# rayanirban/DiffSplitting

Hardware: AMD Instinct MI355X
Metric: sampled images/sec (2000-step 128x128 SR3) (higher is better)
Workload: dtype bf16; 1 GPU; sr_sr3_16_128: GaussianDiffusion.p_sample_loop, 16->128 SR3 UNet (97.8M params), T=2000 linear schedule; one step = UNet forward + posterior update of the batch; batch_per_gpu=16, global_batch=16, image=128x128x3, sample_steps=2000, parallelism=1 independent replicas, final RCCL all-gather, hipgraph=True, streams=1, noise=device Philox4x32-10, weights=random-init, seed 0

## Files before the change

diffsplitting_amd/csrc/dsx_attn.hip:

```cpp
#include "dsx_kernels.h"
#include <type_traits>
#include <utility>

namespace dsx {

typedef __attribute__((ext_vector_type(16))) float f32x16;
typedef __attribute__((ext_vector_type(8))) __bf16 bf16x8_a;
typedef __attribute__((ext_vector_type(8))) _Float16 f16x8_a;

namespace {

template <class F, int... I>
__device__ __forceinline__ __attribute__((always_inline)) void attn_static_for_impl(F&& f, std::integer_sequence<int, I...>) {
  (f(std::integral_constant<int, I>{}), ...);
}
template <int N, class F> __device__ __forceinline__ void attn_static_for(F&& f) {
  attn_static_for_impl(f, std::make_integer_sequence<int, N>{});
}

constexpr int BQ = 32;
constexpr int BK = 128;

template <int ST> struct AttnT;
template <> struct AttnT<0> {
  static constexpr int ES = 4;
  static constexpr int DC = 64;
  static constexpr int VK = 64;
};
template <> struct AttnT<1> { static constexpr int ES = 2; static constexpr int DC = 128; static constexpr int VK = 128; };
template <> struct AttnT<2> { static constexpr int ES = 2; static constexpr int DC = 128; static constexpr int VK = 128; };

__device__ __forceinline__ unsigned pack16(float lo, float hi, std::integral_constant<int, 1>) {
  const __bf16 l = (__bf16)lo, h = (__bf16)hi;
  return (unsigned)__builtin_bit_cast(unsigned short, l) | ((unsigned)__builtin_bit_cast(unsigned short, h) << 16);
}
__device__ __forceinline__ unsigned pack16(float lo, float hi, std::integral_constant<int, 2>) {
  const _Float16 l = (_Float16)lo, h = (_Float16)hi;
  return (unsigned)__builtin_bit_cast(unsigned short, l) | ((unsigned)__builtin_bit_cast(unsigned short, h) << 16);
}

template <int ST>
__device__ __forceinline__ f32x16 mfma16(const uint4 a, const uint4 b, f32x16 c) {
  if constexpr (ST == 1)
    return __builtin_amdgcn_mfma_f32_32x32x16_bf16(__builtin_bit_cast(bf16x8_a, a), __builtin_bit_cast(bf16x8_a, b), c, 0, 0, 0);
  else
    return __builtin_amdgcn_mfma_f32_32x32x16_f16(__builtin_bit_cast(f16x8_a, a), __builtin_bit_cast(f16x8_a, b), c, 0, 0, 0);
}

__device__ __forceinline__ int vt_slot(int row, int slot) { return slot ^ (((row >> 3) ^ row) & 15); }

}

template <int ST, int NDB, int CS>
__global__ __launch_bounds__(256, (NDB <= 1 ? 2 : 1)) void k_attn(const AttnArgs a) {
  static_assert(NDB % CS == 0, "whole chunks per workgroup");
  constexpr int NDO = NDB / CS;
  using T = AttnT<ST>;
  constexpr int ES = T::ES, DC = T::DC, VK = T::VK;
  constexpr bool F32 = ST == 0;
  constexpr int KUNITS = NDB * (128 / DC);
  constexpr int VPC = BK / VK;
  constexpr int VUNITS = NDO * VPC;
  constexpr int KROW = F32 ? (DC + 1) * 4 : DC * 2 + 16;
  constexpr int PROW = F32 ? (BK + 1) * 4 : BK * 2 + 16;
  constexpr int VROW = F32 ? 128 * 4 : BK * 2;
  constexpr int KV_BYTES = (BK * KROW > (F32 ? VK : 128) * VROW) ? BK * KROW : (F32 ? VK : 128) * VROW;
  constexpr int Q_BYTES = BQ * KROW;
  constexpr int P_BYTES = BQ * PROW;

  extern __shared__ __attribute__((aligned(16))) unsigned char smem[];
  unsigned char* kv_lds = smem;
  unsigned char* q_lds = smem + KV_BYTES;
  unsigned char* p_lds = q_lds + Q_BYTES;
  float* red = (float*)(p_lds + P_BYTES);

  const int tid = threadIdx.x, lane = tid & 63;
  const int wave = __builtin_amdgcn_readfirstlane(tid >> 6);
  const int li = lane & 31, lh = lane >> 5;

  const int QT = (a.L + BQ - 1) / BQ;
  const int total = a.B * QT * CS;
  int j = blockIdx.x;
  if ((total & 7) == 0) j = (blockIdx.x & 7) * (total >> 3) + (blockIdx.x >> 3);
  const int half = CS == 1 ? 0 : j % CS;
  const int jq = CS == 1 ? j : j / CS;
  const int b = jq / QT, q0 = (jq - b * QT) * BQ;
  const int chunk0 = half * NDO;

  const size_t row0 = (size_t)b * a.L;
  const size_t ldb = (size_t)a.ld * ES;

  constexpr int SEGS = (DC * ES) / 16;
  static_assert(SEGS == 16, "a staged K/Q row is 256 bytes");
  const int seg = tid & 15, rsub = tid >> 4;
#ifndef DSX_ATTN_PD
#define DSX_ATTN_PD 2
#endif
  constexpr int PD = (KUNITS + VUNITS) < DSX_ATTN_PD ? (KUNITS + VUNITS) : DSX_ATTN_PD;
  uint4 pre[PD][10];

  const __amdgpu_buffer_rsrc_t rs = __builtin_amdgcn_make_buffer_rsrc(
      (void*)((const char*)a.q + row0 * ldb), 0, (int)((size_t)a.L * ldb), 0x00020000);
  const unsigned koff = (unsigned)((const char*)a.k - (const char*)a.q), voff = (unsigned)((const char*)a.v - (const char*)a.q);
  auto ld16 = [&](unsigned tensor_off, int row, int col_elem) __attribute__((always_inline)) -> uint4 {
    const unsigned vo = col_elem < a.C ? (unsigned)row * (unsigned)ldb + tensor_off + (unsigned)col_elem * ES : 0x80000000u;
    return __builtin_bit_cast(uint4, __builtin_amdgcn_raw_buffer_load_b128(rs, vo, 0, 0));
  };

  auto issue_unit = [&](int key0, int u, uint4 (&pre)[10]) __attribute__((always_inline)) {
    if (u < KUNITS) {
      const int c0 = u * DC + seg * (16 / ES);
#pragma unroll
      for (int it = 0; it < 8; ++it) {
        const int key = key0 + rsub + 16 * it;
        pre[it] = ld16(koff, key, c0);
      }
#pragma unroll
      for (int it = 0; it < 2; ++it) {
        const int q = q0 + rsub + 16 * it;
        pre[8 + it] = ld16(0u, q, c0);
      }
    } else {
      const int v = u - KUNITS, chunk = v / VPC, part = v - chunk * VPC;
      if constexpr (F32) {
        const int s32 = tid & 31, r8 = tid >> 5;
        const int c0 = (chunk0 + chunk) * 128 + s32 * 4;
#pragma unroll
        for (int it = 0; it < 8; ++it) {
          const int key = key0 + part * VK + r8 + 8 * it;
          pre[it] = ld16(voff, key, c0);
        }
      } else {
        const int c0 = (chunk0 + chunk) * 128 + seg * 8;
#pragma unroll
        for (int it = 0; it < 4; ++it) {
          const int key = key0 + 2 * (rsub + 16 * it);
          pre[2 * it] = ld16(voff, key, c0);
          pre[2 * it + 1] = ld16(voff, key + 1, c0);
        }
      }
    }
  };
  auto store_unit = [&](int u, const uint4 (&pre)[10]) __attribute__((always_inline)) {
    if (u < KUNITS) {
      auto put = [&](unsigned char* dst, const uint4 v) __attribute__((always_inline)) {
        if constexpr (F32) {
          unsigned* d = (unsigned*)dst;
          d[0] = v.x; d[1] = v.y; d[2] = v.z; d[3] = v.w;
        } else {
          *(uint4*)dst = v;
        }
      };
#pragma unroll
      for (int it = 0; it < 8; ++it) put(kv_lds + (rsub + 16 * it) * KROW + seg * 16, pre[it]);
#pragma unroll
      for (int it = 0; it < 2; ++it) put(q_lds + (rsub + 16 * it) * KROW + seg * 16, pre[8 + it]);
    } else {
      if constexpr (F32) {
        const int s32 = tid & 31, r8 = tid >> 5;
#pragma unroll
        for (int it = 0; it < 8; ++it) *(uint4*)(kv_lds + (r8 + 8 * it) * VROW + s32 * 16) = pre[it];
      } else {
#pragma unroll
        for (int it = 0; it < 4; ++it) {
          const int pair = rsub + 16 * it;
          const unsigned ea[4] = {pre[2 * it].x, pre[2 * it].y, pre[2 * it].z, pre[2 * it].w};
          const unsigned eb[4] = {pre[2 * it + 1].x, pre[2 * it + 1].y, pre[2 * it + 1].z, pre[2 * it + 1].w};
#pragma unroll
          for (int jj = 0; jj < 8; ++jj) {
            const unsigned lo = (jj & 1) ? (ea[jj >> 1] >> 16) : (ea[jj >> 1] & 0xffffu);
            const unsigned hi = (jj & 1) ? (eb[jj >> 1] & 0xffff0000u) : (eb[jj >> 1] << 16);
            const int row = seg * 8 + jj;
            *(unsigned*)(kv_lds + row * VROW + vt_slot(row, pair >> 2) * 16 + (pair & 3) * 4) = lo | hi;
          }
        }
      }
    }
  };

  f32x16 oacc[NDO];
#pragma unroll
  for (int c = 0; c < NDO; ++c)
#pragma unroll
    for (int r = 0; r < 16; ++r) oacc[c][r] = 0.f;
  float m_run = -INFINITY, l_run = 0.f;
  f32x16 sacc;

  const int ntiles = (a.L + BK - 1) / BK;
  constexpr int UPT = KUNITS + VUNITS;
  static_assert(UPT % PD == 0 && UPT >= PD, "the register slot of a unit is a compile-time constant");
  attn_static_for<PD>([&](auto pc) __attribute__((always_inline)) {
    constexpr int u0 = decltype(pc)::value;
    issue_unit(0, u0, pre[u0]);
  });
  for (int t = 0; t < ntiles; ++t) {
    const int key0 = t * BK;
#pragma unroll
    for (int r = 0; r < 16; ++r) sacc[r] = 0.f;
    attn_static_for<UPT>([&](auto uc) __attribute__((always_inline)) {
      constexpr int u = decltype(uc)::value;
      __syncthreads();
      store_unit(u, pre[u % PD]);
      __syncthreads();
      {
        constexpr int nu = (u + PD) % UPT;
        const int nk = (u + PD >= UPT) ? key0 + BK : key0;
        if (nk < a.L) issue_unit(nk, nu, pre[u % PD]);
      }
      if constexpr (u < KUNITS) {
        if constexpr (F32) {
          const float* kr = (const float*)(kv_lds + (wave * 32 + li) * KROW);
          const float* qr = (const float*)(q_lds + li * KROW);
#pragma unroll 8
          for (int s = 0; s < DC / 2; ++s)
            sacc = __builtin_amdgcn_mfma_f32_32x32x2f32(kr[2 * s + lh], qr[2 * s + lh], sacc, 0, 0, 0);
        } else {
          const unsigned char* kr = kv_lds + (wave * 32 + li) * KROW + lh * 16;
          const unsigned char* qr = q_lds + li * KROW + lh * 16;
#pragma unroll
          for (int s = 0; s < DC / 16; ++s)
            sacc = mfma16<ST>(*(const uint4*)(kr + s * 32), *(const uint4*)(qr + s * 32), sacc);
        }
        if constexpr (u == KUNITS - 1) {
          float s[16];
          float mx = -INFINITY;
#pragma unroll
          for (int r = 0; r < 16; ++r) {
            const int key = key0 + wave * 32 + (r & 3) + 8 * (r >> 2) + 4 * lh;
            float v = F32 ? sacc[r] / a.div : sacc[r] * a.inv_div;
            if (key >= a.L) v = -INFINITY;
            s[r] = v;
            mx = fmaxf(mx, v);
          }
          mx = fmaxf(mx, __shfl_xor(mx, 32, 64));
          if (lh == 0) red[wave * 32 + li] = mx;
          __syncthreads();
          const float tmax = fmaxf(fmaxf(red[li], red[32 + li]), fmaxf(red[64 + li], red[96 + li]));
          const float m_new = fmaxf(m_run, tmax);
          const float alpha = F32 ? expf(m_run - m_new) : __expf(m_run - m_new);
          float psum = 0.f;
#pragma unroll
          for (int r = 0; r < 16; ++r) { s[r] = F32 ? expf(s[r] - m_new) : __expf(s[r] - m_new); psum += s[r]; }
          psum += __shfl_xor(psum, 32, 64);
          if (lh == 0) red[128 + wave * 32 + li] = psum;
          if constexpr (F32) {
            float* pr = (float*)(p_lds + li * PROW);
#pragma unroll
            for (int r = 0; r < 16; ++r) pr[wave * 32 + (r & 3) + 8 * (r >> 2) + 4 * lh] = s[r];
          } else {
#pragma unroll
            for (int g = 0; g < 4; ++g) {
              uint2 w;
              w.x = pack16(s[4 * g], s[4 * g + 1], std::integral_constant<int, ST>{});
              w.y = pack16(s[4 * g + 2], s[4 * g + 3], std::integral_constant<int, ST>{});
              *(uint2*)(p_lds + li * PROW + (wave * 32 + 8 * g + 4 * lh) * 2) = w;
            }
          }
          __syncthreads();
          const float tsum = (red[128 + li] + red[160 + li]) + (red[192 + li] + red[224 + li]);
          l_run = l_run * alpha + tsum;
          m_run = m_new;
#pragma unroll
          for (int c = 0; c < NDO; ++c)
#pragma unroll
            for (int r = 0; r < 16; ++r) oacc[c][r] *= alpha;
        }
      } else {
        constexpr int v = u - KUNITS, chunk = v / VPC, part = v - chunk * VPC;
        f32x16 acc = oacc[chunk];
        if constexpr (F32) {
          const float* vr = (const float*)kv_lds + wave * 32 + li;
          const float* pr = (const float*)(p_lds + li * PROW) + part * VK;
#pragma unroll 8
          for (int s = 0; s < VK / 2; ++s)
            acc = __builtin_amdgcn_mfma_f32_32x32x2f32(vr[(2 * s + lh) * 128], pr[2 * s + lh], acc, 0, 0, 0);
        } else {
          const int row = wave * 32 + li;
          const unsigned char* vr = kv_lds + row * VROW;
          const unsigned char* pr = p_lds + li * PROW + lh * 16;
#pragma unroll
          for (int s = 0; s < BK / 16; ++s)
            acc = mfma16<ST>(*(const uint4*)(vr + vt_slot(row, 2 * s + lh) * 16), *(const uint4*)(pr + s * 32), acc);
        }
        oacc[chunk] = acc;
      }
    });
  }

  const int q = q0 + li;
  if (q >= a.L) return;
  const float inv_l = 1.0f / l_run;
  char* orow = (char*)a.out + ((size_t)b * a.L + q) * (size_t)a.ldo * ES;
#pragma unroll
  for (int c = 0; c < NDO; ++c) {
#pragma unroll
    for (int g = 0; g < 4; ++g) {
      const int ch = (chunk0 + c) * 128 + wave * 32 + 8 * g + 4 * lh;
      if (ch >= a.C) continue;
      const float x0 = oacc[c][4 * g] * inv_l, x1 = oacc[c][4 * g + 1] * inv_l;
      const float x2 = oacc[c][4 * g + 2] * inv_l, x3 = oacc[c][4 * g + 3] * inv_l;
      if constexpr (F32) {
        *(float4*)(orow + (size_t)ch * 4) = make_float4(x0, x1, x2, x3);
      } else {
        uint2 w;
        w.x = pack16(x0, x1, std::integral_constant<int, ST>{});
        w.y = pack16(x2, x3, std::integral_constant<int, ST>{});
        *(uint2*)(orow + (size_t)ch * 2) = w;
      }
    }
  }
}

namespace {
template <int ST> constexpr size_t attn_lds_bytes() {
  using T = AttnT<ST>;
  constexpr bool F32 = ST == 0;
  constexpr int KROW = F32 ? (T::DC + 1) * 4 : T::DC * 2 + 16;
  constexpr int PROW = F32 ? (BK + 1) * 4 : BK * 2 + 16;
  constexpr int VROW = F32 ? 128 * 4 : BK * 2;
  constexpr int KV = (BK * KROW > (F32 ? T::VK : 128) * VROW) ? BK * KROW : (F32 ? T::VK : 128) * VROW;
  return (size_t)KV + (size_t)BQ * KROW + (size_t)BQ * PROW + 2 * 4 * 32 * sizeof(float);
}
template <int ST, int NDB, int CS = 1> hipError_t launch_attn_one(const AttnArgs& a, hipStream_t st) {
  const int QT = (a.L + BQ - 1) / BQ;
  hipLaunchKernelGGL((k_attn<ST, NDB, CS>), dim3((unsigned)(a.B * QT * CS)), dim3(256), attn_lds_bytes<ST>(), st, a);
  return hipGetLastError();
}
template <int ST> hipError_t launch_attn_st(const AttnArgs& a, bool col_split, hipStream_t st) {
  const int ndb = (a.C + 127) / 128;
  switch (ndb) {
    case 1: return launch_attn_one<ST, 1>(a, st);
    case 2: return launch_attn_one<ST, 2>(a, st);
    case 3: case 4: {
      const int QT = (a.L + BQ - 1) / BQ;
      if (col_split && a.B * QT <= 160) return launch_attn_one<ST, 4, 2>(a, st);
      return launch_attn_one<ST, 4>(a, st);
    }
    case 5: case 6: case 7: case 8: return launch_attn_one<ST, 8>(a, st);
    default: return hipErrorInvalidValue;
  }
}
}

bool attn_supported(int C, int L) { return C >= 8 && C <= 1024 && (C & 7) == 0 && L >= 1 && (long long)L * 3 * C * 4 < (1LL << 31); }

hipError_t launch_attn(const AttnArgs& a, bool col_split, hipStream_t st) {
  if (!attn_supported(a.C, a.L) || a.B < 1) return hipErrorInvalidValue;
  const int epu = a.storage == 0 ? 4 : 8;
  if ((a.ld % epu) || (a.ldo % 4) || ((uintptr_t)a.q & 15) || ((uintptr_t)a.k & 15) || ((uintptr_t)a.v & 15) ||
      ((uintptr_t)a.out & 15))
    return hipErrorInvalidValue;
  switch (a.storage) {
    case 0: return launch_attn_st<0>(a, col_split, st);
    case 1: return launch_attn_st<1>(a, col_split, st);
    case 2: return launch_attn_st<2>(a, col_split, st);
    default: return hipErrorInvalidValue;
  }
}

}
```

diffsplitting_amd/csrc/dsx_exec.cpp:

```cpp
#include "dsx_rt.h"

std::unique_ptr<dsx_exec> dsx::new_exec(dsx_model* m, int B, int H, int W, int cond_channels) {
  auto ex = std::make_unique<dsx_exec>();
  ex->m = m; ex->B = B; ex->H = H; ex->W = W;
  ex->knobs = read_plan_knobs();
  ex->knobs.conv_naive = m->want_naive;
  ex->cond_c = cond_channels; ex->x_c = m->cfg.in_channel - cond_channels;
  return ex;
}

extern "C" int dsx_exec_create(dsx_model* m, int B, int H, int W, int cond_channels, dsx_exec** out) {
  if (!m || !out || B < 1 || H < 1 || W < 1) return fail(DSX_ERR_INVALID, "bad argument");
  if (!m->finalized) return fail(DSX_ERR_STATE, "dsx_model_finalize must precede dsx_exec_create");
  if (cond_channels < 0 || cond_channels >= m->cfg.in_channel) return fail(DSX_ERR_INVALID, "bad cond_channels");
  HIP_TRY(conv_init());
  HIP_TRY(ops_init());
  auto ex = new_exec(m, B, H, W, cond_channels);
  const int rc = run_planner(ex.get(), nullptr, nullptr);
  if (rc) return rc;
  if (hipMemset(ex->step_ctr, 0, 256) != hipSuccess) return fail(DSX_ERR_HIP, "hipMemset failed");
  *out = ex.release();
  return DSX_OK;
}

static int drop_graph(dsx_exec* ex) {
  if (ex->graph.exec && ex->last_stream) HIP_TRY(hipStreamSynchronize(ex->last_stream));
  ex->graph.reset();
  return DSX_OK;
}

extern "C" void dsx_exec_destroy(dsx_exec* ex) {
  if (!ex) return;
  for (auto& sl : ex->staging)
    if (sl.busy) (void)hipEventSynchronize(sl.ev.e);
  (void)drop_graph(ex);
  delete ex;
}
extern "C" size_t dsx_exec_workspace_bytes(const dsx_exec* ex) { return ex ? ex->ws_bytes : 0; }
extern "C" int dsx_exec_handoff_timeouts(dsx_exec* ex, unsigned* count) {
  if (!ex || !count) return fail(DSX_ERR_INVALID, "null argument");
  HIP_TRY(hipDeviceSynchronize());
  HIP_TRY(hipMemcpy(count, ex->handoff_timeouts, sizeof(unsigned), hipMemcpyDeviceToHost));
  return DSX_OK;
}
extern "C" int dsx_exec_num_launches(const dsx_exec* ex) { return ex ? ex->launches : 0; }

extern "C" int dsx_exec_num_ops(const dsx_exec* ex) { return ex ? (int)ex->ops.size() : 0; }
extern "C" int dsx_exec_num_layers(const dsx_exec* ex) { return ex ? (int)ex->layers.size() : 0; }
extern "C" int dsx_exec_layer_info(const dsx_exec* ex, int i, dsx_layer_info* info) {
  if (!ex || !info || i < 0 || i >= (int)ex->layers.size()) return fail(DSX_ERR_INVALID, "bad layer index");
  *info = ex->layers[i];
  return DSX_OK;
}
extern "C" int dsx_exec_copy_workspace(const dsx_exec* ex, uint64_t src, size_t bytes, void* dst, void* stream) {
  if (!ex || !dst) return fail(DSX_ERR_INVALID, "null argument");
  const uint64_t lo = (uint64_t)(uintptr_t)ex->ws, hi = lo + ex->ws_bytes;
  if (!ex->ws || src < lo || src > hi || bytes > hi - src) return fail(DSX_ERR_INVALID, "range is not inside the workspace");
  HIP_TRY(hipMemcpyAsync(dst, (const void*)(uintptr_t)src, bytes, hipMemcpyDeviceToDevice, (hipStream_t)stream));
  return DSX_OK;
}
extern "C" int dsx_exec_op_info(const dsx_exec* ex, int i, char* desc, int cap, int* kind, double* flops,
                                double* bytes) {
  if (!ex || i < 0 || i >= (int)ex->ops.size()) return fail(DSX_ERR_INVALID, "bad op index");
  const PlanOp& o = ex->ops[i];
  if (desc && cap > 0) snprintf(desc, cap, "%s", o.desc.c_str());
  if (kind) *kind = o.kind;
  if (flops) *flops = o.flops;
  if (bytes) *bytes = o.bytes;
  return DSX_OK;
}
extern "C" int dsx_exec_time_kind(dsx_exec* ex, int kind, int iters, float* ms_per_replay, int* launches,
                                  void* stream) {
  if (!ex || !ms_per_replay || iters < 1) return fail(DSX_ERR_INVALID, "bad argument");
  hipStream_t st = (hipStream_t)stream;
  if (!st) return fail(DSX_ERR_INVALID, "dsx_exec_time_kind needs a non-default stream (stream capture)");
  auto selected = [&](int k) { return kind >= 0 ? k == kind : (kind == -1 ? true : k != -kind - 2); };
  int n = 0;
  for (auto& op : ex->ops) n += selected(op.kind) ? 1 : 0;
  if (launches) *launches = n;
  if (n == 0) { *ms_per_replay = 0.f; return DSX_OK; }
  Graph g;
  HIP_TRY(hipStreamSynchronize(st));
  HIP_TRY(hipStreamBeginCapture(st, hipStreamCaptureModeThreadLocal));
  hipError_t err = hipSuccess;
  for (size_t i = 0; i < ex->ops.size() && err == hipSuccess; ++i)
    if (selected(ex->ops[i].kind)) err = launch_op(ex->ops[i], st);
  hipError_t e2 = hipStreamEndCapture(st, &g.graph);
  if (err != hipSuccess || e2 != hipSuccess || !g.graph)
    return fail(DSX_ERR_HIP, "capture of the kernel family failed: %s", hipGetErrorString(err != hipSuccess ? err : e2));
  HIP_TRY(hipGraphInstantiate(&g.exec, g.graph, nullptr, nullptr, 0));
  Event e0, e1;
  HIP_TRY(e0.create());
  HIP_TRY(e1.create());
  HIP_TRY(hipGraphLaunch(g.exec, st));
  HIP_TRY(hipEventRecord(e0.e, st));
  for (int it = 0; it < iters; ++it) HIP_TRY(hipGraphLaunch(g.exec, st));
  HIP_TRY(hipEventRecord(e1.e, st));
  HIP_TRY(hipStreamSynchronize(st));
  float ms = 0.f;
  HIP_TRY(hipEventElapsedTime(&ms, e0.e, e1.e));
  *ms_per_replay = ms / iters;
  return DSX_OK;
}

extern "C" int dsx_exec_read_stamps(dsx_exec* ex, unsigned long long* out128) {
  if (!ex || !out128) return fail(DSX_ERR_INVALID, "null argument");
  memset(out128, 0, 128 * 8);
  if (!ex->stamp_buf) return DSX_OK;
  HIP_TRY(hipDeviceSynchronize());
  HIP_TRY(hipMemcpy(out128, ex->stamp_buf, 128 * 8, hipMemcpyDeviceToHost));
  return DSX_OK;
}

extern "C" int dsx_exec_profile(dsx_exec* ex, int iters, float* ms_per_op, void* stream) {
  if (!ex || !ms_per_op || iters < 1) return fail(DSX_ERR_INVALID, "bad argument");
  hipStream_t st = (hipStream_t)stream;
  const size_t n = ex->ops.size();
  std::vector<Event> ev(2 * n);
  for (auto& e : ev) HIP_TRY(e.create());
  std::vector<double> acc(n, 0.0);
  for (int it = 0; it < iters; ++it) {
    static const bool trace = getenv("DSX_TRACE") != nullptr;
    for (size_t i = 0; i < n; ++i) {
      if (trace) { fprintf(stderr, "[dsx] op %zu: %s\n", i, ex->ops[i].desc.c_str()); fflush(stderr); }
      HIP_TRY(hipEventRecord(ev[2 * i].e, st));
      HIP_TRY(launch_op(ex->ops[i], st));
      HIP_TRY(hipEventRecord(ev[2 * i + 1].e, st));
      if (trace) HIP_TRY(hipStreamSynchronize(st));
    }
    HIP_TRY(hipStreamSynchronize(st));
    for (size_t i = 0; i < n; ++i) {
      float ms = 0.f;
      HIP_TRY(hipEventElapsedTime(&ms, ev[2 * i].e, ev[2 * i + 1].e));
      acc[i] += ms;
    }
  }
  for (size_t i = 0; i < n; ++i) ms_per_op[i] = (float)(acc[i] / iters);
  return DSX_OK;
}

static int run_unet(dsx_exec* ex, bool from_table, int n_time, hipStream_t st, int per_sample = 0) {
  dsx_model* m = ex->m;
  if (m->cfg.with_time_emb) {
    TembArgs t{};
    t.flavour = m->cfg.flavour; t.B = ex->B; t.n_time = n_time;
    t.time = from_table ? nullptr : ex->time_buf;
    t.table = ex->table.as<float>(); t.step_ctr = ex->step_ctr; t.per_sample = per_sample;
    t.inner = m->cfg.inner_channel; t.freq = m->d_freq;
    t.w1 = m->d_w1; t.b1 = m->d_b1; t.w2 = m->d_w2; t.b2 = m->d_b2;
    t.wf = m->d_wf; t.bf = m->d_bf; t.F = m->F; t.film = ex->film;
    HIP_TRY(launch_temb(t, st));
  }
  for (auto& op : ex->ops) HIP_TRY(launch_op(op, st));
  return DSX_OK;
}

static int load_inputs(dsx_exec* ex, const float* cond_nchw, const float* x_nchw, int x_total_c,
                       int x_c_off, hipStream_t st);

extern "C" int dsx_unet_forward(dsx_exec* ex, const float* x, const float* time, int n_time, float* y,
                                void* stream) {
  if (!ex || !x || !y) return fail(DSX_ERR_INVALID, "null argument");
  hipStream_t st = (hipStream_t)stream;
  dsx_model* m = ex->m;
  if (m->cfg.with_time_emb) {
    if (!time || !(n_time == 1 || n_time == ex->B)) return fail(DSX_ERR_INVALID, "n_time must be 1 or B");
    HIP_TRY(hipMemcpyAsync(ex->time_buf, time, (size_t)n_time * 4, hipMemcpyDeviceToDevice, st));
  }
  int rc = load_inputs(ex, ex->cond_c ? x : nullptr, x, m->cfg.in_channel, ex->cond_c, st);
// ... 258 lines not shown
```

diffsplitting_amd/csrc/dsx_kernels.h:

```cpp
#pragma once
#include <hip/hip_runtime.h>
#include <stdint.h>

namespace dsx {

struct PrefetchArgs {
  const void* base;
  unsigned slice_bytes;
  int nslices;
  unsigned* sink;
};
inline unsigned fastdiv_magic(unsigned d) { return d <= 1 ? 0u : (unsigned)((1ull << 32) / d) + 1u; }
#if defined(__HIPCC__)
__device__ __forceinline__ unsigned fastdiv(unsigned n, unsigned magic) { return magic ? __umulhi(n, magic) : n; }
struct PfAcc { unsigned v[4]; };
__device__ __forceinline__ PfAcc l2_prefetch(const PrefetchArgs& pf, unsigned lin_block, unsigned nblocks_total, int tid, int nthreads) {
  PfAcc acc = {{0u, 0u, 0u, 0u}};
  if (pf.base == nullptr || pf.nslices <= 0) return acc;
  const unsigned label = lin_block & 7u, j = lin_block >> 3, n8 = (nblocks_total + 7u) >> 3;
  const unsigned lines = pf.slice_bytes >> 7;
  const unsigned per = (lines + n8 - 1u) / n8, l0 = j * per;
  const unsigned l1 = l0 + per < lines ? l0 + per : lines;
  const int s0 = pf.nslices < 8 ? (int)(label % (unsigned)pf.nslices) : (int)label;
  const int sstep = pf.nslices < 8 ? pf.nslices : 8;
// ... 100 lines not shown
#pragma unroll
    for (int w = 0; w < NW; ++w) { s += red[2 * w]; q += red[2 * w + 1]; }
  }
  const double n = a.count * cpg;
  const double mean = s / n;
  double var = q / n - mean * mean;
  if (var < 0) var = 0;
  const float rstd = (float)(1.0 / sqrt(var + (double)a.eps));
  const float meanf = (float)mean;
  if (own) {
    const float sc = rstd * g_own;
    a.scale[(size_t)b * C + c_own] = sc;
    a.shift[(size_t)b * C + c_own] = b_own - meanf * sc;
  }
  for (int c = c_lo + tid + NT; c < c_lo + cpg; c += NT) {
    const float sc = rstd * a.gamma[c];
    a.scale[(size_t)b * C + c] = sc;
    a.shift[(size_t)b * C + c] = a.beta[c] - meanf * sc;
  }
}
#endif

struct ConvArgs {
  const void* src0;
  const void* src1;
  int act_bf16;
  int out_bf16;
  int C0, C1;
  int B, Hs, Ws;
  int up;
  int Ho, Wo;
  const float* gn_scale;
  const float* gn_shift;
  int has_gn;
  int swish;
  int stage_mode;
  const void* wpack;
  const float* bias;
  const float* film;
  int film_bs;
  const void* resid;
  int resid_ld;
  void* out;
  int out_ld;
  int Cout;
  int nblocks;
  int kchunks;
  int tw_log2, th_log2, tb_log2;
  int tiles_x, tiles_y, m_tiles, n_tiles;
  int lds_row;
  int cpg;
  int ws_wg_per_n;
  int ws_cpg;
  int xcd_bands;
  int ws_map;
  int ws_nt_log2;
  int ws_per;
  int ws_adv_x, ws_adv_y, ws_adv_b;
  int ws_dpy, ws_dpx;
  unsigned mg_tiles_x, mg_per_img, mg_pw, mg_wpn, mg_per;
  int ws_bigdiv;
  float* stat_part;
  unsigned* handoff_timeouts;
  unsigned long long* stamp;
  int stamp_block;
  int ablate;
  const void* gn_part0; int gn_nchunk0, gn_pf32_0;
  const void* gn_part1; int gn_nchunk1, gn_pf32_1;
  StatPivot gn_piv0, gn_piv1;
  const float* gn_gamma; const float* gn_beta;
  int gn_groups; float gn_eps;
  PrefetchArgs pf;
  int fin_on;
  GnFinArgs fin;
  int ksplit;
  int groups_per_split;
  long long slab_stride;
};

enum ConvTile { TILE_256x128 = 0, TILE_128x128, TILE_64x128, TILE_256x64, TILE_128x64, TILE_64x64, TILE_128x32, TILE_256x32, TILE_COUNT };
struct ConvTileInfo { int BM, BN, WM; bool fuses_stats; };
ConvTileInfo conv_tile_info(int tile, bool ws = false);
int conv_chunk_multiple(int ks);
constexpr int conv_lds_row(int ks, int stride, int tw_log2, int cpg) {
  const int pixb = 64 * cpg + 16;
  const int pw = ((1 << tw_log2) - 1) * stride + ks;
  int rb = (pw * pixb + 15) & ~15;
  if (ks == 1 || stride != 1) return rb;
  if (tw_log2 == 4) rb = (rb + 255) & ~255;
  else if (tw_log2 == 3) { rb = (rb + 127) & ~127; if (((rb >> 7) & 1) == 0) rb += 128; }
  return rb;
}
size_t conv_lds_bytes(int dtype, int tile, int ks, int stride, const ConvArgs& a);
hipError_t launch_conv(int dtype, int tile, int ks, int stride, const ConvArgs& a, hipStream_t st);
size_t conv_ws_lds_bytes(int dtype, int tile, int ks, const ConvArgs& a);
hipError_t launch_conv_ws(int dtype, int tile, int ks, const ConvArgs& a, hipStream_t st);
bool conv_img_applicable(int dtype, int ks, int stride, const ConvArgs& a, bool gn, int gn_groups);
hipError_t launch_conv_img(int dtype, int ks, const ConvArgs& a, hipStream_t st);
bool conv_first_applicable(int ks, int stride, const ConvArgs& a, bool gn);
hipError_t launch_conv_first(int dtype, const ConvArgs& a, hipStream_t st);
hipError_t conv_init();
hipError_t ops_init();

struct NaiveConvArgs {
  ConvArgs c;
  const float* w;
  int ks, stride;
  int sigmoid_out;
};
hipError_t launch_conv_naive(const NaiveConvArgs& a, hipStream_t st);

hipError_t launch_chan_stats(const void* x, int bf16, int B, int HW, int C, int nchunk, double* part,
                             hipStream_t st);
hipError_t launch_gn_finalize(const GnFinArgs& a, hipStream_t st);

struct TembArgs {
  int flavour;
  int B;
  int n_time;
  const float* time;
  const float* table;
  const int* step_ctr;
  int per_sample;
  int inner;
  const float* freq;
  const float* w1; const float* b1;
  const float* w2; const float* b2;
  const float* wf; const float* bf;
  int F;
  float* film;
};
hipError_t launch_temb(const TembArgs& a, hipStream_t st);

struct SplitKReduceArgs {
  const float* slab; int nsplit; long long slab_stride;
  long long M; int N; int HW;
  const float* bias; const float* film; int film_bs;
  const void* resid; int resid_ld;
  void* out;
  int act_bf16;
  float* stat_part;
};
hipError_t launch_splitk_reduce(const SplitKReduceArgs& a, hipStream_t st);

struct AttnArgs {
  const void* q; const void* k; const void* v; int ld;
  void* out; int ldo;
  int storage;
  int B, L, C;
  float div, inv_div;
};
bool attn_supported(int C, int L);
hipError_t launch_attn(const AttnArgs& a, bool col_split, hipStream_t st);

hipError_t launch_nchw_slice_to_nhwc(const float* src, void* dst, int dst_bf16, int B, int C, int ctot, int coff,
                                     int HW, hipStream_t st);
hipError_t launch_nhwc_to_nchw(const float* src, float* dst, int B, int C, int H, int W, hipStream_t st);

struct UpdateArgs {
  float* x;
  void* x_act;
  int x_act_kind;
  const float* net;
  int use_noise;
  const unsigned long long* loop_params;
  const float* tab;
  int n_steps;
  const int* step_ctr;
  int predict_eps, clip;
  int per_sample;
  int B, C, H, W;
};
hipError_t launch_update(const UpdateArgs& a, hipStream_t st);
hipError_t launch_advance(int* step_ctr, hipStream_t st);
hipError_t launch_randn(float* out, long long n, unsigned long long seed, unsigned long long subseq,
                        hipStream_t st);
static inline unsigned grid_for(long long total) {
  long long g = (total + 255) / 256;
  return (unsigned)(g > 4096 ? 4096 : (g < 1 ? 1 : g));
}
#if defined(__HIPCC__)
__device__ __forceinline__ float mul_f(float a, float b) {
#pragma clang fp contract(off)
  return a * b;
}
__device__ __forceinline__ float add_f(float a, float b) {
#pragma clang fp contract(off)
  return a + b;
}
__device__ __forceinline__ float sub_f(float a, float b) {
#pragma clang fp contract(off)
  return a - b;
}
__device__ __forceinline__ double mul_d(double a, double b) {
#pragma clang fp contract(off)
  return a * b;
}
__device__ __forceinline__ double add_d(double a, double b) {
#pragma clang fp contract(off)
  return a + b;
}

struct StepVals { float x0, mean, out; };
__device__ __forceinline__ StepVals step_update(float a, float b, float c1, float c2, float sigma, bool predict_eps,
                                                bool clip, float x, float net, float z, bool use_z) {
  StepVals v;
  v.x0 = net;
  if (predict_eps) {
    v.x0 = sub_f(mul_f(a, x), mul_f(b, net));
    if (clip) v.x0 = fminf(fmaxf(v.x0, -1.0f), 1.0f);
  }
  v.mean = add_f(mul_f(c1, v.x0), mul_f(c2, x));
  v.out = use_z ? add_f(v.mean, mul_f(z, sigma)) : v.mean;
  return v;
}

__device__ __forceinline__ void philox4x32_10(unsigned c0, unsigned c1, unsigned c2, unsigned c3,
                                              unsigned k0, unsigned k1, unsigned out[4]) {
#pragma unroll
  for (int r = 0; r < 10; ++r) {
    const unsigned long long p0 = (unsigned long long)0xD2511F53u * c0;
    const unsigned long long p1 = (unsigned long long)0xCD9E8D57u * c2;
    const unsigned n0 = (unsigned)(p1 >> 32) ^ c1 ^ k0;
    const unsigned n1 = (unsigned)p1;
    const unsigned n2 = (unsigned)(p0 >> 32) ^ c3 ^ k1;
    const unsigned n3 = (unsigned)p0;
    c0 = n0; c1 = n1; c2 = n2; c3 = n3;
    k0 += 0x9E3779B9u; k1 += 0xBB67AE85u;
  }
  out[0] = c0; out[1] = c1; out[2] = c2; out[3] = c3;
}
__device__ __forceinline__ void normal4(unsigned long long seed, unsigned long long subseq,
                                        unsigned long long idx4, float z[4]) {
  unsigned r[4];
  philox4x32_10((unsigned)idx4, (unsigned)(idx4 >> 32), (unsigned)subseq, (unsigned)(subseq >> 32),
                (unsigned)seed, (unsigned)(seed >> 32), r);
  const float u0 = ((float)r[0] + 0.5f) * 2.3283064365386963e-10f;
  const float u1 = ((float)r[1] + 0.5f) * 2.3283064365386963e-10f;
  const float u2 = ((float)r[2] + 0.5f) * 2.3283064365386963e-10f;
  const float u3 = ((float)r[3] + 0.5f) * 2.3283064365386963e-10f;
  const float ra = sqrtf(-2.0f * logf(u0)), rb = sqrtf(-2.0f * logf(u2));
  float s, c;
  sincosf(6.283185307179586f * u1, &s, &c);
  z[0] = ra * c; z[1] = ra * s;
  sincosf(6.283185307179586f * u3, &s, &c);
  z[2] = rb * c; z[3] = rb * s;
}
#endif

struct QSampleArgs {
  const float* x0; const float* xe;
  const float* c0; const float* c1; const float* c2;
  const float* z; unsigned long long seed, subseq; float* z_out;
  float* dst;
  int B, C, Ce, HW, Cdst, coff;
};
hipError_t launch_q_sample(const QSampleArgs& a, hipStream_t st);
int loss_blocks(long long n);
hipError_t launch_loss(const float* a, const float* b, int B, long long n, int squared, double* part, double* out,
                       hipStream_t st);

struct PosteriorStepArgs {
  const float* x; const float* net;
  const float* a; const float* b; const float* c1; const float* c2; const float* sigma;
  const float* z; unsigned long long seed, subseq;
  float* x_recon_out; float* mean_out; float* x_out;
  int B, predict_eps, clip, repeat;
  long long CHW;
};
hipError_t launch_posterior_step(const PosteriorStepArgs& a, long long HW, hipStream_t st);
struct InterpStartArgs {
  const float* x1; const float* x2; const float* a0; const float* s0;
  const float* z1; const float* z2; unsigned long long seed, subseq;
  float c, d;
  float* out;
  int B;
  long long CHW;
};
hipError_t launch_interp_start(const InterpStartArgs& a, long long HW, hipStream_t st);

struct TileSeq { long long first, stride, count; };
hipError_t launch_tiles_gather(const float* frames, int H, int W, int ph, int pw, const int* starts , TileSeq seq,
                               float* tiles, hipStream_t st);
hipError_t launch_tiles_gather_norm(const float* f0, const float* f1, int H, int W, int ph, int pw, const int* starts,
                                    TileSeq seq, float w0, float w1, const double norm[6], int from_norm_target,
                                    float* tin, float* ttar, hipStream_t st);
struct MixWeights { float w0, w1, lo0, rng0, lo1, rng1; };
hipError_t launch_tiles_gather_mix(const float* f0, const float* f1, int H, int W, int ph, int pw, const int* starts,
                                   TileSeq seq, const double norm[4], const MixWeights& mw, float* ttar, float* tmix,
                                   float* tcls, hipStream_t st);
int mix_range_blocks(long long pixels);
hipError_t launch_mix_range(const float* f0, const float* f1, long long pixels, const double norm[4], int n, double* part,
                            hipStream_t st);
struct StitchSrc {
  const float* base; int packed; int ph, pw;
  const long long* off; long long rank_stride; int world;
};
hipError_t launch_stitch(const StitchSrc& s, int C, const int* regions , TileSeq seq, float* canvas, int H, int W,
                         const float* gt, double* part, int gx, hipStream_t st);
hipError_t launch_tiles_pack(const float* tiles, int C, int ph, int pw, const int* regions, const long long* off,
                             TileSeq seq, float* flat, hipStream_t st);

struct SsimWindow { double w[11]; };
int image_metrics_tiles(int H, int W);
hipError_t launch_image_metrics(const float* a, const float* b, int planes, int H, int W, int quantize, float lo,
                                float hi, float rng, double c1, double c2, const SsimWindow& win, double* part,
// ... 36 lines not shown
```

Baseline: 2.967 images/s.

## Add short-sequence attention kernel with double-buffered LDS and transposed V reads

Adds a specialized 16-bit attention kernel for sequences of at most two key tiles. It keeps the whole Q block resident in LDS, double-buffers K/V units through two LDS slots with register prefetch, and reads V via ds_read_tr16 transposed loads instead of the generic path. The shared softmax and output-store code is factored into helpers, and an init hook raises the dynamic LDS limit. This trades one workgroup per CU for less staging overhead on short attention calls in the SR3 UNet (low-resolution levels).

Result: no change. 2.992 images/s, median of 6 (+0.8%).

```diff
diff --git a/diffsplitting_amd/csrc/dsx_attn.hip b/diffsplitting_amd/csrc/dsx_attn.hip
--- a/diffsplitting_amd/csrc/dsx_attn.hip
+++ b/diffsplitting_amd/csrc/dsx_attn.hip
@@ -1,4 +1,5 @@
 #include "dsx_kernels.h"
+#include <mutex>
 #include <type_traits>
 #include <utility>
 
@@ -48,6 +49,95 @@
 }
 
 __device__ __forceinline__ int vt_slot(int row, int slot) { return slot ^ (((row >> 3) ^ row) & 15); }
+
+template <int NDB> struct AttnShortLds {
+  static constexpr int KROW = 128 * 2 + 16;
+  static constexpr int VROW = 128 * 2 + 64;
+  static constexpr int QROW = NDB * 256 + 16;
+  static constexpr int PROW = BK * 2 + 16;
+  static constexpr int SLOT = BK * (KROW > VROW ? KROW : VROW);
+  static constexpr size_t BYTES = 2 * (size_t)SLOT + (size_t)BQ * QROW + (size_t)BQ * PROW + 2 * 4 * 32 * sizeof(float);
+  static_assert(BYTES <= 160 * 1024, "one workgroup per CU");
+};
+
+typedef __attribute__((ext_vector_type(4))) short i16x4_a;
+__device__ __forceinline__ uint2 lds_read_tr16(const unsigned char* p) {
+  return __builtin_bit_cast(uint2, __builtin_amdgcn_ds_read_tr16_b64_v4i16((__attribute__((address_space(3))) i16x4_a*)p));
+}
+
+template <int ST>
+__device__ __forceinline__ float attn_softmax_tile(const AttnArgs& a, const f32x16& sacc, int key0, int wave, int li, int lh,
+                                                   float* red, unsigned char* p_lds, int PROW, float& m_run, float& l_run) {
+  constexpr bool F32 = ST == 0;
+  float s[16];
+  float mx = -INFINITY;
+#pragma unroll
+  for (int r = 0; r < 16; ++r) {
+    const int key = key0 + wave * 32 + (r & 3) + 8 * (r >> 2) + 4 * lh;
+    float v = F32 ? sacc[r] / a.div : sacc[r] * a.inv_div;
+    if (key >= a.L) v = -INFINITY;
+    s[r] = v;
+    mx = fmaxf(mx, v);
+  }
+  mx = fmaxf(mx, __shfl_xor(mx, 32, 64));
+  if (lh == 0) red[wave * 32 + li] = mx;
+  __syncthreads();
+  const float tmax = fmaxf(fmaxf(red[li], red[32 + li]), fmaxf(red[64 + li], red[96 + li]));
+  const float m_new = fmaxf(m_run, tmax);
+  const float alpha = F32 ? expf(m_run - m_new) : __expf(m_run - m_new);
+  float psum = 0.f;
+#pragma unroll
+  for (int r = 0; r < 16; ++r) { s[r] = F32 ? expf(s[r] - m_new) : __expf(s[r] - m_new); psum += s[r]; }
+  psum += __shfl_xor(psum, 32, 64);
+  if (lh == 0) red[128 + wave * 32 + li] = psum;
+  if constexpr (F32) {
+    float* pr = (float*)(p_lds + li * PROW);
+#pragma unroll
+    for (int r = 0; r < 16; ++r) pr[wave * 32 + (r & 3) + 8 * (r >> 2) + 4 * lh] = s[r];
+  } else {
+#pragma unroll
+    for (int g = 0; g < 4; ++g) {
+      uint2 w;
+      w.x = pack16(s[4 * g], s[4 * g + 1], std::integral_constant<int, ST>{});
+      w.y = pack16(s[4 * g + 2], s[4 * g + 3], std::integral_constant<int, ST>{});
+      *(uint2*)(p_lds + li * PROW + (wave * 32 + 8 * g + 4 * lh) * 2) = w;
+    }
+  }
+  __syncthreads();
+  const float tsum = (red[128 + li] + red[160 + li]) + (red[192 + li] + red[224 + li]);
+  l_run = l_run * alpha + tsum;
+  m_run = m_new;
+  return alpha;
+}
+
+template <int ST, int NDO>
+__device__ __forceinline__ void attn_store_out(const AttnArgs& a, const f32x16 (&oacc)[NDO], float l_run, int b, int q0,
+                                               int chunk0, int wave, int li, int lh) {
+  constexpr bool F32 = ST == 0;
+  constexpr int ES = AttnT<ST>::ES;
+  const int q = q0 + li;
+  if (q >= a.L) return;
+  const float inv_l = 1.0f / l_run;
+  char* orow = (char*)a.out + ((size_t)b * a.L + q) * (size_t)a.ldo * ES;
+#pragma unroll
+  for (int c = 0; c < NDO; ++c) {
+#pragma unroll
+    for (int g = 0; g < 4; ++g) {
+      const int ch = (chunk0 + c) * 128 + wave * 32 + 8 * g + 4 * lh;
+      if (ch >= a.C) continue;
+      const float x0 = oacc[c][4 * g] * inv_l, x1 = oacc[c][4 * g + 1] * inv_l;
+      const float x2 = oacc[c][4 * g + 2] * inv_l, x3 = oacc[c][4 * g + 3] * inv_l;
+      if constexpr (F32) {
+        *(float4*)(orow + (size_t)ch * 4) = make_float4(x0, x1, x2, x3);
+      } else {
+        uint2 w;
+        w.x = pack16(x0, x1, std::integral_constant<int, ST>{});
+        w.y = pack16(x2, x3, std::integral_constant<int, ST>{});
+        *(uint2*)(orow + (size_t)ch * 2) = w;
+      }
+    }
+  }
+}
 
 }
 
@@ -93,10 +183,7 @@
   constexpr int SEGS = (DC * ES) / 16;
   static_assert(SEGS == 16, "a staged K/Q row is 256 bytes");
   const int seg = tid & 15, rsub = tid >> 4;
-#ifndef DSX_ATTN_PD
-#define DSX_ATTN_PD 2
-#endif
-  constexpr int PD = (KUNITS + VUNITS) < DSX_ATTN_PD ? (KUNITS + VUNITS) : DSX_ATTN_PD;
+  constexpr int PD = 2;
   uint4 pre[PD][10];
 
   const __amdgpu_buffer_rsrc_t rs = __builtin_amdgcn_make_buffer_rsrc(
@@ -222,44 +309,7 @@
             sacc = mfma16<ST>(*(const uint4*)(kr + s * 32), *(const uint4*)(qr + s * 32), sacc);
         }
         if constexpr (u == KUNITS - 1) {
-          float s[16];
-          float mx = -INFINITY;
-#pragma unroll
-          for (int r = 0; r < 16; ++r) {
-            const int key = key0 + wave * 32 + (r & 3) + 8 * (r >> 2) + 4 * lh;
-            float v = F32 ? sacc[r] / a.div : sacc[r] * a.inv_div;
-            if (key >= a.L) v = -INFINITY;
-            s[r] = v;
-            mx = fmaxf(mx, v);
-          }
-          mx = fmaxf(mx, __shfl_xor(mx, 32, 64));
-          if (lh == 0) red[wave * 32 + li] = mx;
-          __syncthreads();
-          const float tmax = fmaxf(fmaxf(red[li], red[32 + li]), fmaxf(red[64 + li], red[96 + li]));
-          const float m_new = fmaxf(m_run, tmax);
-          const float alpha = F32 ? expf(m_run - m_new) : __expf(m_run - m_new);
-          float psum = 0.f;
-#pragma unroll
-          for (int r = 0; r < 16; ++r) { s[r] = F32 ? expf(s[r] - m_new) : __expf(s[r] - m_new); psum += s[r]; }
-          psum += __shfl_xor(psum, 32, 64);
-          if (lh == 0) red[128 + wave * 32 + li] = psum;
-          if constexpr (F32) {
-            float* pr = (float*)(p_lds + li * PROW);
-#pragma unroll
-            for (int r = 0; r < 16; ++r) pr[wave * 32 + (r & 3) + 8 * (r >> 2) + 4 * lh] = s[r];
-          } else {
-#pragma unroll
-            for (int g = 0; g < 4; ++g) {
-              uint2 w;
-              w.x = pack16(s[4 * g], s[4 * g + 1], std::integral_constant<int, ST>{});
-              w.y = pack16(s[4 * g + 2], s[4 * g + 3], std::integral_constant<int, ST>{});
-              *(uint2*)(p_lds + li * PROW + (wave * 32 + 8 * g + 4 * lh) * 2) = w;
-            }
-          }
-          __syncthreads();
-          const float tsum = (red[128 + li] + red[160 + li]) + (red[192 + li] + red[224 + li]);
-          l_run = l_run * alpha + tsum;
-          m_run = m_new;
+          const float alpha = attn_softmax_tile<ST>(a, sacc, key0, wave, li, lh, red, p_lds, PROW, m_run, l_run);
 #pragma unroll
           for (int c = 0; c < NDO; ++c)
 #pragma unroll
@@ -287,30 +337,126 @@
     });
   }
 
-  const int q = q0 + li;
-  if (q >= a.L) return;
-  const float inv_l = 1.0f / l_run;
-  char* orow = (char*)a.out + ((size_t)b * a.L + q) * (size_t)a.ldo * ES;
-#pragma unroll
-  for (int c = 0; c < NDO; ++c) {
-#pragma unroll
-    for (int g = 0; g < 4; ++g) {
-      const int ch = (chunk0 + c) * 128 + wave * 32 + 8 * g + 4 * lh;
-      if (ch >= a.C) continue;
-      const float x0 = oacc[c][4 * g] * inv_l, x1 = oacc[c][4 * g + 1] * inv_l;
-      const float x2 = oacc[c][4 * g + 2] * inv_l, x3 = oacc[c][4 * g + 3] * inv_l;
-      if constexpr (F32) {
-        *(float4*)(orow + (size_t)ch * 4) = make_float4(x0, x1, x2, x3);
+  attn_store_out<ST, NDO>(a, oacc, l_run, b, q0, chunk0, wave, li, lh);
+}
+
+template <int ST, int NDB, int CS>
+__global__ __launch_bounds__(256, 1) void k_attn_short(const AttnArgs a) {
+  static_assert(ST != 0 && NDB % CS == 0, "16-bit operands; whole chunks per workgroup");
+  constexpr int NDO = NDB / CS;
+  constexpr int ES = 2;
+  constexpr int KROW = AttnShortLds<NDB>::KROW, VROW = AttnShortLds<NDB>::VROW, QROW = AttnShortLds<NDB>::QROW;
+  constexpr int PROW = AttnShortLds<NDB>::PROW, SLOT = AttnShortLds<NDB>::SLOT;
+  constexpr int KUNITS = NDB, VUNITS = NDO, UPT = KUNITS + VUNITS;
+  static_assert(UPT % 2 == 0, "the LDS slot and the register set of a unit are compile-time constants");
+
+  extern __shared__ __attribute__((aligned(16))) unsigned char smem[];
+  unsigned char* q_lds = smem + 2 * SLOT;
+  unsigned char* p_lds = q_lds + BQ * QROW;
+  float* red = (float*)(p_lds + BQ * PROW);
+
+  const int tid = threadIdx.x, lane = tid & 63;
+  const int wave = __builtin_amdgcn_readfirstlane(tid >> 6);
+  const int li = lane & 31, lh = lane >> 5;
+
+  const int QT = (a.L + BQ - 1) / BQ;
+  const int total = a.B * QT * CS;
+  int j = blockIdx.x;
+  if ((total & 7) == 0) j = (blockIdx.x & 7) * (total >> 3) + (blockIdx.x >> 3);
+  const int half = CS == 1 ? 0 : j % CS;
+  const int jq = CS == 1 ? j : j / CS;
+  const int b = jq / QT, q0 = (jq - b * QT) * BQ;
+  const int chunk0 = half * NDO;
+
+  const size_t row0 = (size_t)b * a.L;
+  const size_t ldb = (size_t)a.ld * ES;
+  const int seg = tid & 15, rsub = tid >> 4;
+
+  const __amdgpu_buffer_rsrc_t rs = __builtin_amdgcn_make_buffer_rsrc(
+      (void*)((const char*)a.q + row0 * ldb), 0, (int)((size_t)a.L * ldb), 0x00020000);
+  const unsigned koff = (unsigned)((const char*)a.k - (const char*)a.q), voff = (unsigned)((const char*)a.v - (const char*)a.q);
+  auto ld16 = [&](unsigned tensor_off, int row, int col_elem) __attribute__((always_inline)) -> uint4 {
+    const unsigned vo = col_elem < a.C ? (unsigned)row * (unsigned)ldb + tensor_off + (unsigned)col_elem * ES : 0x80000000u;
+    return __builtin_bit_cast(uint4, __builtin_amdgcn_raw_buffer_load_b128(rs, vo, 0, 0));
+  };
+  auto issue_unit = [&](int key0, int u, uint4 (&pre)[8]) __attribute__((always_inline)) {
+    const unsigned toff = u < KUNITS ? koff : voff;
+    const int c0 = (u < KUNITS ? u : chunk0 + (u - KUNITS)) * 128 + seg * 8;
+#pragma unroll
+    for (int it = 0; it < 8; ++it) pre[it] = ld16(toff, key0 + rsub + 16 * it, c0);
+  };
+  auto store_unit = [&](int u, const uint4 (&pre)[8]) __attribute__((always_inline)) {
+    unsigned char* dst = smem + (u & 1) * SLOT + seg * 16;
+    const int pitch = u < KUNITS ? KROW : VROW;
+#pragma unroll
+    for (int it = 0; it < 8; ++it) *(uint4*)(dst + (rsub + 16 * it) * pitch) = pre[it];
+  };
+
+  const int ntiles = (a.L + BK - 1) / BK;
+  uint4 pre[2][8];
+  {
+    uint4 qreg[2 * NDB];
+#pragma unroll
+    for (int it = 0; it < 2 * NDB; ++it) qreg[it] = ld16(0u, q0 + rsub + 16 * (it & 1), (it >> 1) * 128 + seg * 8);
+    issue_unit(0, 0, pre[0]);
+    issue_unit(0, 1, pre[1]);
+#pragma unroll
+    for (int it = 0; it < 2 * NDB; ++it)
+      *(uint4*)(q_lds + (rsub + 16 * (it & 1)) * QROW + (it >> 1) * 256 + seg * 16) = qreg[it];
+    store_unit(0, pre[0]);
+    if (UPT > 2 || ntiles > 1) issue_unit(UPT > 2 ? 0 : BK, 2 % UPT, pre[0]);
+  }
+  __syncthreads();
+
+  f32x16 oacc[NDO];
+#pragma unroll
+  for (int c = 0; c < NDO; ++c)
+#pragma unroll
+    for (int r = 0; r < 16; ++r) oacc[c][r] = 0.f;
+  float m_run = -INFINITY, l_run = 0.f;
+  f32x16 sacc;
+
+  const int vtr = (8 * (lane >> 5) + ((lane >> 2) & 3)) * VROW + (wave * 32 + 16 * ((lane >> 4) & 1) + 4 * (lane & 3)) * 2;
+
+  for (int t = 0; t < ntiles; ++t) {
+    const int key0 = t * BK;
+    const bool more = t + 1 < ntiles;
+#pragma unroll
+    for (int r = 0; r < 16; ++r) sacc[r] = 0.f;
+    attn_static_for<UPT>([&](auto uc) __attribute__((always_inline)) {
+      constexpr int u = decltype(uc)::value;
+      if (u + 1 < UPT || more) store_unit((u + 1) % UPT, pre[(u + 1) & 1]);
+      constexpr int ahead = (u + 3) / UPT;
+      if (t + ahead < ntiles) issue_unit(key0 + ahead * BK, (u + 3) % UPT, pre[(u + 1) & 1]);
+      const unsigned char* slot = smem + (u & 1) * SLOT;
+      if constexpr (u < KUNITS) {
+        const unsigned char* kr = slot + (wave * 32 + li) * KROW + lh * 16;
+        const unsigned char* qr = q_lds + li * QROW + u * 256 + lh * 16;
+#pragma unroll
+        for (int s = 0; s < 8; ++s)
+          sacc = mfma16<ST>(*(const uint4*)(kr + s * 32), *(const uint4*)(qr + s * 32), sacc);
+        if constexpr (u == KUNITS - 1) {
+          const float alpha = attn_softmax_tile<ST>(a, sacc, key0, wave, li, lh, red, p_lds, PROW, m_run, l_run);
+#pragma unroll
+          for (int c = 0; c < NDO; ++c)
+#pragma unroll
+            for (int r = 0; r < 16; ++r) oacc[c][r] *= alpha;
+        }
       } else {
-        uint2 w;
-        w.x = pack16(x0, x1, std::integral_constant<int, ST>{});
-        w.y = pack16(x2, x3, std::integral_constant<int, ST>{});
-        *(uint2*)(orow + (size_t)ch * 2) = w;
-      }
-    }
-  }
-}
-
+        f32x16 acc = oacc[u - KUNITS];
+        const unsigned char* pr = p_lds + li * PROW + lh * 16;
+#pragma unroll
+        for (int s = 0; s < 8; ++s) {
+          const uint2 lo = lds_read_tr16(slot + vtr + s * 16 * VROW), hi = lds_read_tr16(slot + vtr + (s * 16 + 4) * VROW);
+          acc = mfma16<ST>(make_uint4(lo.x, lo.y, hi.x, hi.y), *(const uint4*)(pr + s * 32), acc);
+        }
+        oacc[u - KUNITS] = acc;
+      }
+      __syncthreads();
+    });
+  }
+  attn_store_out<ST, NDO>(a, oacc, l_run, b, q0, chunk0, wave, li, lh);
+}
 namespace {
 template <int ST> constexpr size_t attn_lds_bytes() {
   using T = AttnT<ST>;
@@ -323,8 +469,27 @@
 }
 template <int ST, int NDB, int CS = 1> hipError_t launch_attn_one(const AttnArgs& a, hipStream_t st) {
   const int QT = (a.L + BQ - 1) / BQ;
-  hipLaunchKernelGGL((k_attn<ST, NDB, CS>), dim3((unsigned)(a.B * QT * CS)), dim3(256), attn_lds_bytes<ST>(), st, a);
+  const dim3 grid((unsigned)(a.B * QT * CS));
+  if constexpr (ST != 0) {
+    if (a.L <= 2 * BK) {
+      hipLaunchKernelGGL((k_attn_short<ST, NDB, CS>), grid, dim3(256), AttnShortLds<NDB>::BYTES, st, a);
+      return hipGetLastError();
+    }
+  }
+  hipLaunchKernelGGL((k_attn<ST, NDB, CS>), grid, dim3(256), attn_lds_bytes<ST>(), st, a);
   return hipGetLastError();
+}
+template <int ST, int NDB, int CS> hipError_t attn_init_one() {
+  return hipFuncSetAttribute((const void*)k_attn_short<ST, NDB, CS>, hipFuncAttributeMaxDynamicSharedMemorySize,
+                             (int)AttnShortLds<NDB>::BYTES);
+}
+template <int ST> hipError_t attn_init_st() {
+  hipError_t e = attn_init_one<ST, 1, 1>();
+  if (e == hipSuccess) e = attn_init_one<ST, 2, 1>();
+  if (e == hipSuccess) e = attn_init_one<ST, 4, 1>();
+  if (e == hipSuccess) e = attn_init_one<ST, 4, 2>();
+  if (e == hipSuccess) e = attn_init_one<ST, 8, 1>();
+  return e;
 }
 template <int ST> hipError_t launch_attn_st(const AttnArgs& a, bool col_split, hipStream_t st) {
   const int ndb = (a.C + 127) / 128;
@@ -344,6 +509,17 @@
 
 bool attn_supported(int C, int L) { return C >= 8 && C <= 1024 && (C & 7) == 0 && L >= 1 && (long long)L * 3 * C * 4 < (1LL << 31); }
 
+hipError_t attn_init() {
+  static std::mutex mu;
+  static bool done = false;
+  std::lock_guard<std::mutex> lock(mu);
+  if (done) return hipSuccess;
+  hipError_t e = attn_init_st<1>();
+  if (e == hipSuccess) e = attn_init_st<2>();
+  done = e == hipSuccess;
+  return e;
+}
+
 hipError_t launch_attn(const AttnArgs& a, bool col_split, hipStream_t st) {
   if (!attn_supported(a.C, a.L) || a.B < 1) return hipErrorInvalidValue;
   const int epu = a.storage == 0 ? 4 : 8;
diff --git a/diffsplitting_amd/csrc/dsx_exec.cpp b/diffsplitting_amd/csrc/dsx_exec.cpp
--- a/diffsplitting_amd/csrc/dsx_exec.cpp
+++ b/diffsplitting_amd/csrc/dsx_exec.cpp
@@ -15,6 +15,7 @@
   if (cond_channels < 0 || cond_channels >= m->cfg.in_channel) return fail(DSX_ERR_INVALID, "bad cond_channels");
   HIP_TRY(conv_init());
   HIP_TRY(ops_init());
+  HIP_TRY(attn_init());
   auto ex = new_exec(m, B, H, W, cond_channels);
   const int rc = run_planner(ex.get(), nullptr, nullptr);
   if (rc) return rc;
diff --git a/diffsplitting_amd/csrc/dsx_kernels.h b/diffsplitting_amd/csrc/dsx_kernels.h
--- a/diffsplitting_amd/csrc/dsx_kernels.h
+++ b/diffsplitting_amd/csrc/dsx_kernels.h
@@ -276,6 +276,7 @@
 };
 bool attn_supported(int C, int L);
 hipError_t launch_attn(const AttnArgs& a, bool col_split, hipStream_t st);
+hipError_t attn_init();
 
 hipError_t launch_nchw_slice_to_nhwc(const float* src, void* dst, int dst_bf16, int B, int C, int ctot, int coff,
                                      int HW, hipStream_t st);
```
